# Pixie8888/R3DFSSeg

Hardware: AMD Instinct MI355X
Metric: episodes/sec S3DIS 2-way 5-shot 2048-pt (MPTI+attention, train step: forward+backward+grad all-reduce+Adam) (higher is better)
Workload: dtype f32 (index-free GEMMs -- self-attention, 1x1 convolutions, weight gradients, the EdgeConv backward's edge GEMMs -- as bf16x3 split products on the bf16 MFMA with fp32 accumulate; every index-deciding result: fp32)

## Files before the change

r3dfsseg_amd/csrc/head_graph.hip:

```cpp
#include "common.h"

#define HG_NC 4
typedef unsigned short hg_col_t;
#define HG_ROWS_PER_BLOCK_MIN 4
#define HG_MAX_PART 2048

struct HgEp {
  long nodes, nbr, y, z, g, lam, dn;
  long desc;
  long ws;
  long stats;
  long labels, logits, loss, pred;
};
#define HG_WS(p) p = (decltype(p))((const char*)(p) + (long)ep * st.ws * 4)
#define HG_AT(p, stride) p += (long)ep * (stride)

__global__ __launch_bounds__(256) void r3d_graph_bits_kernel(const int* __restrict__ nbr, int kp1, const int* __restrict__ n_dev,
                                                             int n_cap, int words, unsigned* __restrict__ outb, HgEp st) {
  __shared__ unsigned bm[4][1024];
  const int ep = blockIdx.y;
  nbr += (long)ep * st.nbr * kp1; HG_AT(n_dev, st.desc); HG_WS(outb);
  const int n = min(*n_dev, n_cap);
  const int w = threadIdx.x >> 6, lane = threadIdx.x & 63;
  const int i = blockIdx.x * 4 + w;
  unsigned* b = bm[w];
  for (int wd = lane; wd < words; wd += 64) b[wd] = 0u;
  __syncthreads();
  if (i < n) {
    const int k = kp1 - 1;
    for (int t = lane; t < k; t += 64) {
      const int j = nbr[(long)i * kp1 + 1 + t];
      if (j < 0 || j >= n || j == i) continue;
      atomicOr(&b[j >> 5], 1u << (j & 31));
    }
  }
  __syncthreads();
  if (i < n_cap)
    for (int wd = lane; wd < words; wd += 64) outb[(long)i * words + wd] = b[wd];
}

#define BT_ROWS 1024
#define BT_CW 8
__global__ __launch_bounds__(256) void r3d_graph_transpose_kernel(const unsigned* __restrict__ outb, int words, int n_cap,
                                                                  unsigned* __restrict__ inb ,
                                                                  HgEp st) {
  __shared__ unsigned tile[BT_CW * 32][BT_ROWS / 32 + 1];
  const int ep = blockIdx.z;
  HG_WS(outb); HG_WS(inb);
  const int c0w = blockIdx.x * BT_CW, r0 = blockIdx.y * BT_ROWS;
  const int w = threadIdx.x >> 6, lane = threadIdx.x & 63;
  for (int sb = w; sb < BT_ROWS / 64; sb += 4) {
    const int r = r0 + sb * 64 + lane;
    unsigned v[BT_CW];
#pragma unroll
    for (int cw = 0; cw < BT_CW; ++cw) v[cw] = (r < n_cap && c0w + cw < words) ? outb[(long)r * words + c0w + cw] : 0u;
#pragma unroll
    for (int cw = 0; cw < BT_CW; ++cw) {
#pragma unroll
      for (int b = 0; b < 32; ++b) {
        const unsigned long long m = __ballot((v[cw] >> b) & 1u);
        if (lane == b) {
          tile[cw * 32 + b][2 * sb] = (unsigned)m;
          tile[cw * 32 + b][2 * sb + 1] = (unsigned)(m >> 32);
        }
      }
    }
  }
  __syncthreads();
  for (int e = threadIdx.x; e < BT_CW * 32 * (BT_ROWS / 32); e += 256) {
    const int c = e >> 5, wd = e & 31;
    const int col = c0w * 32 + c, ow = r0 / 32 + wd;
    if (col < n_cap && ow < words) inb[(long)col * words + ow] = tile[c][wd];
  }
}

__global__ void r3d_graph_rowlen_kernel(unsigned* __restrict__ sym ,
                                        const unsigned* __restrict__ outb, int words,
                                        const int* __restrict__ n_dev, int n_cap, int* __restrict__ row_len, HgEp st) {
  const int ep = blockIdx.y;
  HG_WS(sym); HG_WS(outb); HG_AT(n_dev, st.desc); HG_WS(row_len);
  const int n = min(*n_dev, n_cap);
  const int row = blockIdx.x * (blockDim.x >> 6) + (threadIdx.x >> 6);
  const int lane = threadIdx.x & 63;
  if (row >= n_cap) return;
  int c = 0;
  if (row < n)
    for (int wd = lane; wd < words; wd += 64) {
      const unsigned v = sym[(long)row * words + wd] | outb[(long)row * words + wd];
      sym[(long)row * words + wd] = v;
      c += __popc(v);
    }
#pragma unroll
  for (int o = 32; o > 0; o >>= 1) c += __shfl_xor(c, o);
  if (lane == 0) row_len[row] = c;
}

__global__ __launch_bounds__(1024) void r3d_scan_kernel(const int* __restrict__ in, int n, int* __restrict__ out, HgEp st) {
  const int ep = blockIdx.x;
  HG_WS(in); HG_WS(out);
  __shared__ int wave_tot[16];
  __shared__ int carry_s;
  const int tid = threadIdx.x, lane = tid & 63, w = tid >> 6;
  if (tid == 0) carry_s = 0;
  __syncthreads();
  for (int t0 = 0; t0 < n; t0 += 1024) {
    const int i = t0 + tid;
    const int v = i < n ? in[i] : 0;
    int x = v;
#pragma unroll
    for (int o = 1; o < 64; o <<= 1) {
      const int y = __shfl_up(x, o);
      if (lane >= o) x += y;
    }
    if (lane == 63) wave_tot[w] = x;
    __syncthreads();
    int wbase = 0, tot = 0;
    for (int q = 0; q < 16; ++q) {
      const int tv = wave_tot[q];
      if (q < w) wbase += tv;
      tot += tv;
    }
    const int carry = carry_s;
    if (i < n) out[i] = carry + wbase + x - v;
    __syncthreads();
    if (tid == 0) carry_s = carry + tot;
    __syncthreads();
  }
  if (tid == 0) out[n] = carry_s;
}

__global__ __launch_bounds__(256) void r3d_graph_cols_kernel(const unsigned* __restrict__ sym, int words,
                                                             const int* __restrict__ n_dev, int n_cap,
                                                             const int* __restrict__ row_ptr, hg_col_t* __restrict__ col,
                                                             HgEp st) {
  const int ep = blockIdx.y;
  HG_WS(sym); HG_AT(n_dev, st.desc); HG_WS(row_ptr); HG_WS(col);
  const int n = min(*n_dev, n_cap);
  const int i = blockIdx.x * 4 + (threadIdx.x >> 6);
  const int lane = threadIdx.x & 63;
  if (i >= n) return;
  const int wpl = (words + 63) / 64;
  const int w0 = lane * wpl;
  int mycount = 0;
  for (int t = 0; t < wpl; ++t) {
    const int wd = w0 + t;
    if (wd < words) mycount += __popc(sym[(long)i * words + wd]);
  }
  int incl = mycount;
#pragma unroll
  for (int o = 1; o < 64; o <<= 1) {
    const int y = __shfl_up(incl, o);
    if (lane >= o) incl += y;
  }
  int wpos = row_ptr[i] + incl - mycount;
  for (int t = 0; t < wpl; ++t) {
    const int wd = w0 + t;
    if (wd >= words) break;
    unsigned bits = sym[(long)i * words + wd];
    while (bits) {
      const int b = __ffs((int)bits) - 1;
      bits &= bits - 1;
      col[wpos++] = (hg_col_t)(wd * 32 + b);
    }
  }
}

__global__ __launch_bounds__(256) void r3d_graph_weights_kernel(
    const float* __restrict__ nodes, long ldn, int D, const unsigned* __restrict__ outb, int words,
    const int* __restrict__ n_dev, int n_cap, const int* __restrict__ row_ptr, const hg_col_t* __restrict__ col,
    float sigma, float* __restrict__ val, float* __restrict__ dinv, float* __restrict__ wdir , HgEp st) {
  __shared__ __attribute__((aligned(16))) float xs[256];
  __shared__ float wsum[4];
  const int ep = blockIdx.y;
  nodes += (long)ep * st.nodes * ldn; HG_WS(outb); HG_AT(n_dev, st.desc); HG_WS(row_ptr); HG_WS(col); HG_WS(val); HG_WS(dinv);
  HG_WS(wdir);
  const int n = min(*n_dev, n_cap);
  const int w = threadIdx.x >> 6;
  const int i = blockIdx.x;
  const int lane = threadIdx.x & 63;
  if (i >= n) return;
  const float* xi = nodes + (long)i * ldn;
  xs[threadIdx.x] = (int)threadIdx.x < D ? xi[threadIdx.x] : 0.f;
  __syncthreads();
  const int beg = row_ptr[i], end = row_ptr[i + 1];
  const int D4 = D >> 2;
  const int part = lane & 7, slot = lane >> 3;
  float dsum = 0.f;
  for (int e0 = beg + 8 * w; e0 < end; e0 += 32) {
    const int e = e0 + slot;
    const bool ok = e < end;
    const int j = col[min(e, end - 1)];
    const float* xj = nodes + (long)j * ldn;
    float a = 0.f, b = 0.f;
    auto step = [&](const float4 y, int c4) {
      const float4 x = *reinterpret_cast<const float4*>(&xs[4 * c4]);
      float d1, d2;
      d1 = (x.x - y.x) + 1e-6f; d2 = (y.x - x.x) + 1e-6f; a = __builtin_fmaf(d1, d1, a); b = __builtin_fmaf(d2, d2, b);
      d1 = (x.y - y.y) + 1e-6f; d2 = (y.y - x.y) + 1e-6f; a = __builtin_fmaf(d1, d1, a); b = __builtin_fmaf(d2, d2, b);
      d1 = (x.z - y.z) + 1e-6f; d2 = (y.z - x.z) + 1e-6f; a = __builtin_fmaf(d1, d1, a); b = __builtin_fmaf(d2, d2, b);
      d1 = (x.w - y.w) + 1e-6f; d2 = (y.w - x.w) + 1e-6f; a = __builtin_fmaf(d1, d1, a); b = __builtin_fmaf(d2, d2, b);
    };
    int c4 = part;
    for (; c4 + 40 < D4; c4 += 48) {
      float4 y[6];
#pragma unroll
      for (int u = 0; u < 6; ++u) y[u] = *reinterpret_cast<const float4*>(xj + 4 * (c4 + 8 * u));
#pragma unroll
      for (int u = 0; u < 6; ++u) step(y[u], c4 + 8 * u);
    }
    for (; c4 < D4; c4 += 8) step(*reinterpret_cast<const float4*>(xj + 4 * c4), c4);
    if (part == 0) {
      for (int c = 4 * D4; c < D; ++c) {
        const float y = xj[c], x = xs[c];
        const float d1 = (x - y) + 1e-6f, d2 = (y - x) + 1e-6f;
        a = __builtin_fmaf(d1, d1, a);
        b = __builtin_fmaf(d2, d2, b);
      }
    }
    a = r3d_sum8_dpp(a);
    b = r3d_sum8_dpp(b);
    const bool out_ij = (outb[(long)i * words + (j >> 5)] >> (j & 31)) & 1u;
    const bool out_ji = (outb[(long)j * words + (i >> 5)] >> (i & 31)) & 1u;
    float wij = 0.f, wji = 0.f;
    if (out_ij) { const float d = sqrtf(a) / sigma; wij = expf(-0.5f * (d * d)); }
    if (out_ji) { const float d = sqrtf(b) / sigma; wji = expf(-0.5f * (d * d)); }
    const float wgt = wij + wji;
    if (ok && part == 0) {
      val[e] = wgt;
      *reinterpret_cast<float2*>(wdir + 2L * e) = make_float2(wij, wji);
      dsum += wgt;
    }
  }
  dsum = r3d_wave_sum(dsum);
  if (lane == 0) wsum[w] = dsum;
  __syncthreads();
  if (threadIdx.x == 0)
    dinv[i] = sqrtf(1.0f / ((((wsum[0] + wsum[1]) + wsum[2]) + wsum[3]) + 2.220446049250313e-16f));
}

__global__ void r3d_graph_normalize_kernel(const int* __restrict__ row_ptr, const hg_col_t* __restrict__ col,
                                           const float* __restrict__ dinv, const int* __restrict__ n_dev,
                                           int n_cap, float* __restrict__ val, HgEp st) {
  const int ep = blockIdx.y;
  HG_WS(row_ptr); HG_WS(col); HG_WS(dinv); HG_AT(n_dev, st.desc); HG_WS(val);
  const int n = min(*n_dev, n_cap);
  const int i = blockIdx.x * 4 + (threadIdx.x >> 6);
  const int lane = threadIdx.x & 63;
  if (i >= n) return;
  const float di = dinv[i];
  for (int e = row_ptr[i] + lane; e < row_ptr[i + 1]; e += 64) val[e] = (di * val[e]) * dinv[col[e]];
}

#define HG_MAX_ITER 1022
#define HG_M 64
#define HG_UROWS 256
#define HG_EBLOCKS 16
#define HG_PART (4 + 2 * HG_M * HG_NC)
static_assert(HG_M == 64 && HG_M * HG_NC == 256, "the CG kernels map (aggregate, column) onto 256 threads, aggregate = lane");
struct CgState {
  int done;
  int iters;
  unsigned ticket;
  unsigned ticket_k;
  float bb[HG_NC];
  float rz[HG_NC];
  float beta[HG_NC];
  float mu[HG_M * HG_NC];
  int fail;
  int pad_;
  unsigned long long pub[HG_M * HG_NC + HG_NC + 1];
};
#define CG_PUB_BETA (HG_M * HG_NC)
#define CG_PUB_CONV (HG_M * HG_NC + HG_NC)
#define CG_SPIN_LIMIT (1 << 18)
static_assert(offsetof(CgState, pub) % 8 == 0 && sizeof(CgState) % 4 == 0, "CgState: the published words are 8-byte words");

static __device__ __forceinline__ float4 f4_zero() { return make_float4(0.f, 0.f, 0.f, 0.f); }

static __device__ __forceinline__ float4 block_sum4(float4 v, float4* sm ) {
  const int lane = threadIdx.x & 63, w = threadIdx.x >> 6;
#pragma unroll
  for (int o = 32; o > 0; o >>= 1) {
    v.x += __shfl_xor(v.x, o); v.y += __shfl_xor(v.y, o);
    v.z += __shfl_xor(v.z, o); v.w += __shfl_xor(v.w, o);
  }
  __syncthreads();
  if (lane == 0) sm[w] = v;
  __syncthreads();
  const float4* sh = sm + (w & ~3);
  float4 r = sh[0];
  for (int q = 1; q < 4; ++q) { r.x += sh[q].x; r.y += sh[q].y; r.z += sh[q].z; r.w += sh[q].w; }
  return r;
}

static __device__ __forceinline__ float4 reduce_partials(const float4* part, int nblk, float4* sm) {
  float4 a = f4_zero();
  for (int q0 = threadIdx.x & 255; q0 < nblk; q0 += 8 * 256) {
    float4 p[8];
#pragma unroll
    for (int u = 0; u < 8; ++u) {
      const int q = q0 + 256 * u;
      const bool ok = q < nblk;
      p[u] = part[min(q, nblk - 1)];
      p[u].x = r3d_keep(p[u].x, ok); p[u].y = r3d_keep(p[u].y, ok); p[u].z = r3d_keep(p[u].z, ok); p[u].w = r3d_keep(p[u].w, ok);
    }
#pragma unroll
    for (int u = 0; u < 8; ++u) { a.x += p[u].x; a.y += p[u].y; a.z += p[u].z; a.w += p[u].w; }
  }
  return block_sum4(a, sm);
}

static __device__ __forceinline__ float f4_get(const float4& v, int c) { return c == 0 ? v.x : c == 1 ? v.y : c == 2 ? v.z : v.w; }

#define HG_SEED_PITCH 257
__global__ __launch_bounds__(256) void r3d_cg_aggregate_kernel(const float* __restrict__ nodes, long ldn, int D,
                                                               const int* __restrict__ n_dev, const int* __restrict__ n_proto_dev,
                                                               int n_cap, int rows_per_wave, int* __restrict__ agg, HgEp st) {
  extern __shared__ float smem[];
  {
    const int ep = blockIdx.y;
    nodes += (long)ep * st.nodes * ldn; HG_AT(n_dev, st.desc); HG_AT(n_proto_dev, st.desc); HG_WS(agg);
  }
  const int pitch = D | 1;
  float* seeds = smem;
  float* xrow = smem + HG_M * pitch + (threadIdx.x >> 6) * D;
  const int n = min(*n_dev, n_cap);
  const int n_proto = max(1, min(*n_proto_dev, n));
  const int lane = threadIdx.x & 63, w = threadIdx.x >> 6;
  {
    const int D4 = D >> 2;
    for (int s0 = 0; s0 < HG_M; s0 += 16) {
      const int sd = s0 + (threadIdx.x >> 4), l16 = threadIdx.x & 15;
      const int src = (int)(((long)sd * (n_proto - 1)) / (HG_M - 1));
      const float4* row = reinterpret_cast<const float4*>(nodes + (long)src * ldn);
      float4 v[4];
#pragma unroll
      for (int u = 0; u < 4; ++u) v[u] = row[min(l16 + 16 * u, D4 - 1)];
#pragma unroll
      for (int u = 0; u < 4; ++u) {
        const int c4 = l16 + 16 * u;
        if (c4 < D4) {
          float* dst = seeds + sd * pitch + 4 * c4;
          dst[0] = v[u].x; dst[1] = v[u].y; dst[2] = v[u].z; dst[3] = v[u].w;
        }
      }
    }
  }
  const int row0 = (blockIdx.x * 4 + w) * rows_per_wave;
  float xr[4][4];
#pragma unroll
  for (int k = 0; k < 4; ++k)
#pragma unroll
    for (int u = 0; u < 4; ++u)
      xr[k][u] = nodes[(long)min(row0 + min(k, rows_per_wave - 1), n - 1) * ldn + min(lane + 64 * u, D - 1)];
  __syncthreads();
  for (int k = 0; k < rows_per_wave; ++k) {
    const int i = row0 + k;
    if (i >= n) break;
#pragma unroll
    for (int u = 0; u < 4; ++u)
      if (lane + 64 * u < D) xrow[lane + 64 * u] = k == 0 ? xr[0][u] : k == 1 ? xr[1][u] : k == 2 ? xr[2][u] : xr[3][u];
    float d2 = 0.f;
    const float* sp = seeds + lane * pitch;
    for (int c0 = 0; c0 < D; c0 += 16) {
      float xs_[16], ss_[16];
#pragma unroll
      for (int c = 0; c < 16; ++c) { xs_[c] = xrow[min(c0 + c, D - 1)]; ss_[c] = sp[min(c0 + c, D - 1)]; }
#pragma unroll
      for (int c = 0; c < 16; ++c) {
        const float df = c0 + c < D ? xs_[c] - ss_[c] : 0.f;
        d2 = __builtin_fmaf(df, df, d2);
      }
    }
    unsigned long long key = ((unsigned long long)__float_as_uint(d2) << 32) | (unsigned)lane;
#pragma unroll
    for (int o = 32; o > 0; o >>= 1) {
      const unsigned long long other = __shfl_xor(key, o);
      key = other < key ? other : key;
    }
    if (lane == 0) agg[i] = (int)(key & 63u);
    __builtin_amdgcn_wave_barrier();
  }
}

__global__ __launch_bounds__(256) void r3d_cg_mw_kernel(const int* __restrict__ row_ptr, const hg_col_t* __restrict__ col,
                                                        const float* __restrict__ val, const float* __restrict__ dinv,
                                                        const int* __restrict__ agg, const int* __restrict__ n_dev, int n_cap,
                                                        float alpha_lp, int rows_per_wave, float* __restrict__ MW, HgEp st) {
  __shared__ float2 pairs[4][256];
  {
// ... 788 lines not shown
      const int i = row_of(trow);
      const float4 beta = beta_s;
      const float4 ri = rs[i], pi = p[i], qi = q[i];
      if (fused) r[i] = ri;
      const float u = 1.f / dinv[i];
      const float4 m = mu_s[agg[i]];
      const float4 pn = make_float4((ri.x + u * m.x) + beta.x * pi.x, (ri.y + u * m.y) + beta.y * pi.y,
                                    (ri.z + u * m.z) + beta.z * pi.z, (ri.w + u * m.w) + beta.w * pi.w);
      const float4 qn = make_float4((ri.x + tot.x) + beta.x * qi.x, (ri.y + tot.y) + beta.y * qi.y,
                                    (ri.z + tot.z) + beta.z * qi.z, (ri.w + tot.w) + beta.w * qi.w);
      p[i] = pn;
      q[i] = qn;
      acc_pq = make_float4(pn.x * qn.x, pn.y * qn.y, pn.z * qn.z, pn.w * qn.w);
    }
    pq_s[SL_WAVES * trow + w] = acc_pq;
    __syncthreads();
    if (tid < SL_PASS_ROWS / 4) {
      const float4 a = pq_s[4 * tid], b2 = pq_s[4 * tid + 1], c2 = pq_s[4 * tid + 2], d2 = pq_s[4 * tid + 3];
      const float4 t = make_float4(((a.x + b2.x) + c2.x) + d2.x, ((a.y + b2.y) + c2.y) + d2.y, ((a.z + b2.z) + c2.z) + d2.z,
                                   ((a.w + b2.w) + c2.w) + d2.w);
      const int gidx = (c0 + tid) * n_wg + bx;
      if (gidx < n_part) part_pq[gidx] = t;
    }
    __syncthreads();
  }
}

#ifdef CG_STAMPS
__device__ unsigned long long g_cg_dbg[32];
#define CSTAMP(i) do { if (it == 3 && threadIdx.x == 0 && blockIdx.x == 0) g_cg_dbg[i] = __builtin_amdgcn_s_memtime(); } while (0)
#define CSTAMP_LAST(i) do { if (it == 3 && threadIdx.x == 0) g_cg_dbg[16 + i] = __builtin_amdgcn_s_memtime(); } while (0)
extern "C" int r3d_cg_debug_read(unsigned long long* out32) {
  return hipMemcpyFromSymbol(out32, HIP_SYMBOL(g_cg_dbg), sizeof(g_cg_dbg)) == hipSuccess ? 0 : 1;
}
#else
#define CSTAMP(i)
#define CSTAMP_LAST(i)
#endif

__global__ __launch_bounds__(256) void r3d_cg_update_kernel(
    const int* __restrict__ n_dev, int n_cap, int it, int nblk_pq, const float* __restrict__ dinv, const int* __restrict__ agg,
    const float* __restrict__ MW, const float4* __restrict__ p, const float4* __restrict__ q, float4* __restrict__ x,
    float4* __restrict__ r, const float4* __restrict__ part_pq, float* __restrict__ part, const float* __restrict__ Einv,
    float tol2, CgState* __restrict__ cg, HgEp st, long x_stride) {
  __shared__ float4 sm[4];
  __shared__ float4 rs[HG_UROWS];
  __shared__ float us[HG_UROWS];
  __shared__ int ag[HG_UROWS];
  __shared__ float4 wpart[2 * 4 * HG_M];
  __shared__ double d_s[HG_M * HG_NC];
  __shared__ float t_s[HG_M * HG_NC];
  __shared__ float rr_s[HG_NC];
  __shared__ int last_s;
  {
    const int ep = blockIdx.y;
    HG_AT(n_dev, st.desc); HG_WS(dinv); HG_WS(agg); HG_WS(MW); HG_WS(p); HG_WS(q); HG_AT(x, x_stride); HG_WS(r); HG_WS(part_pq);
    HG_WS(part); HG_WS(Einv); HG_WS(cg);
  }
  if (cg->done | cg->fail) return;
  if (it < 0) it = cg->iters;
  const int row0 = blockIdx.x * HG_UROWS;
  const int i = row0 + threadIdx.x;
  const int ic = min(i, n_cap - 1);
  float m[64];
  CSTAMP(0);
  cg_load_mw_column(MW, row0, n_cap, m);
  const float4 pi = p[ic], qi = q[ic];
  float4 xi = x[ic], ri = r[ic];
  const float dv = dinv[ic];
  const int av = agg[ic];
  const float4 rz = *reinterpret_cast<const float4*>(cg->rz);
  const int n = min(*n_dev, n_cap);
  const float4 pq = reduce_partials(part_pq, nblk_pq, sm);
  CSTAMP(1);
  float4 al;
  al.x = pq.x > 0.f ? rz.x / pq.x : 0.f;
  al.y = pq.y > 0.f ? rz.y / pq.y : 0.f;
  al.z = pq.z > 0.f ? rz.z / pq.z : 0.f;
  al.w = pq.w > 0.f ? rz.w / pq.w : 0.f;
  float u = 0.f;
  int a = 0;
  if (i < n) {
    xi.x += al.x * pi.x; xi.y += al.y * pi.y; xi.z += al.z * pi.z; xi.w += al.w * pi.w;
    ri.x -= al.x * qi.x; ri.y -= al.y * qi.y; ri.z -= al.z * qi.z; ri.w -= al.w * qi.w;
    x[i] = xi; r[i] = ri;
    u = 1.f / dv;
    a = av;
  } else {
    ri = f4_zero();
  }
  rs[threadIdx.x] = ri; us[threadIdx.x] = u; ag[threadIdx.x] = a;
  __syncthreads();
  CSTAMP(2);
  cg_block_partials(rs, us, ag, row0, n, m, true, part + (long)blockIdx.x * HG_PART, sm, wpart);
  CSTAMP(3);
  const bool last = cg_delivered_last(cg, gridDim.x, &last_s);
  CSTAMP(4);
  if (last) {
    CSTAMP_LAST(0);
    cg_reduce_step<false>(part, gridDim.x, Einv, 1, it + 1, tol2, cg, d_s, t_s, rr_s);
    CSTAMP_LAST(1);
  }
}

__global__ __launch_bounds__(1024) void r3d_logits_ce_kernel(const float4* __restrict__ Z, const float4* __restrict__ Z2,
                                                             const int* __restrict__ desc_nproto, int n_q, int N, int n_classes,
                                                             const long long* __restrict__ labels,
                                                             float* __restrict__ logits ,
                                                             float* __restrict__ loss_out, int* __restrict__ pred_out, HgEp st) {
  __shared__ float red[16];
  {
    const int ep = blockIdx.x;
    HG_AT(Z, st.z); HG_AT(desc_nproto, st.desc); HG_AT(logits, st.logits);
    if (Z2) HG_AT(Z2, st.z);
    if (labels) HG_AT(labels, st.labels);
    if (loss_out) HG_AT(loss_out, st.loss);
    if (pred_out) HG_AT(pred_out, st.pred);
  }
  const int n_proto = *desc_nproto;
  float acc = 0.f;
  for (int e = threadIdx.x; e < n_q * N; e += blockDim.x) {
    const int qi = e / N, p = e - qi * N;
    const float4 z = Z[n_proto + e];
    const float4 z2 = Z2 ? Z2[n_proto + e] : f4_zero();
    const float zv[8] = {z.x, z.y, z.z, z.w, z2.x, z2.y, z2.z, z2.w};
    float mx = zv[0];
    int am = 0;
    for (int c = 1; c < n_classes; ++c) if (zv[c] > mx) { mx = zv[c]; am = c; }
    float se = 0.f;
    for (int c = 0; c < n_classes; ++c) {
      logits[((long)qi * n_classes + c) * N + p] = zv[c];
      se += expf(zv[c] - mx);
    }
    if (labels) {
      const int lab = (int)labels[e];
      acc += (mx + logf(se)) - zv[lab];
    }
    if (pred_out) pred_out[e] = am;
  }
  acc = r3d_wave_sum(acc);
  if ((threadIdx.x & 63) == 0) red[threadIdx.x >> 6] = acc;
  __syncthreads();
  if (threadIdx.x == 0) {
    float t = 0.f;
    for (int w = 0; w < (int)(blockDim.x >> 6); ++w) t += red[w];
    if (loss_out) *loss_out = t / (float)(n_q * N);
  }
}

struct LpWs {
  unsigned *outb, *sym;
  int *row_len, *row_ptr, *agg;
  hg_col_t* col;
  float *val, *dinv, *wdir, *MW, *Epart, *part;
  float* Einv;
  float4 *r, *p, *q, *part_pq;
  CgState* cg;
  long words, total;
};

static inline long hg_vblocks(int n_cap) { return r3d_cdiv(n_cap, HG_UROWS); }

static LpWs lp_carve(int32_t* ws, int n_cap, int kp1) {
  LpWs L;
  L.words = (n_cap + 31) / 32;
  const long nnz_cap = 2L * n_cap * (kp1 - 1);
  int32_t* wp = ws;
  auto align4 = [&]() { wp += (4 - ((wp - ws) & 3)) & 3; };
  L.outb = (unsigned*)wp; wp += n_cap * L.words;
  L.sym = (unsigned*)wp; wp += n_cap * L.words;
  L.row_len = wp; wp += n_cap + 8;
  L.row_ptr = wp; wp += n_cap + 8;
  L.col = (hg_col_t*)wp; wp += (nnz_cap + 1) / 2;
  L.val = (float*)wp; wp += nnz_cap;
  L.wdir = (float*)wp; wp += 2 * nnz_cap;
  L.dinv = (float*)wp; wp += n_cap;
  L.agg = wp; wp += n_cap;
  align4();
  L.MW = (float*)wp; wp += (long)n_cap * HG_M;
  L.Epart = (float*)wp; wp += (long)HG_EBLOCKS * HG_M * HG_M;
  align4();
  L.Einv = (float*)wp; wp += (long)HG_M * HG_M;
  L.part = (float*)wp; wp += hg_vblocks(n_cap) * HG_PART;
  align4();
  L.r = (float4*)wp; wp += 4L * n_cap;
  L.p = (float4*)wp; wp += 4L * n_cap;
  L.q = (float4*)wp; wp += 4L * n_cap;
  L.part_pq = (float4*)wp; wp += 4L * HG_MAX_PART;
  L.cg = (CgState*)wp; wp += (sizeof(CgState) + 3) / 4;
  L.total = (wp - ws) + 64;
  return L;
}

extern "C" long r3d_lp_ws_words(int n_cap, int kp1) { return lp_carve(nullptr, n_cap, kp1).total; }

extern "C" int r3d_lp_ws_offsets(int n_cap, int kp1, long* out6) {
  R3D_REQUIRE(out6 && n_cap > 0 && kp1 >= 2, "r3d_lp_ws_offsets: bad arguments");
  const LpWs L = lp_carve(nullptr, n_cap, kp1);
  const int32_t* base = nullptr;
  out6[0] = (const int32_t*)L.row_ptr - base; out6[1] = (const int32_t*)L.col - base; out6[2] = (const int32_t*)L.val - base;
  out6[3] = (const int32_t*)L.dinv - base; out6[4] = (const int32_t*)L.agg - base; out6[5] = (const int32_t*)L.cg - base;
  return R3D_OK;
}

__global__ void r3d_weights_compare_kernel(const int* __restrict__ row_ptr, const int* __restrict__ n_dev, int n_cap,
                                           const float* __restrict__ wdir, const float* __restrict__ wdir2, long scratch_stride,
                                           int* __restrict__ mismatch, HgEp st) {
  const int ep = blockIdx.y;
  HG_WS(row_ptr); HG_AT(n_dev, st.desc); HG_WS(wdir);
  wdir2 += (long)ep * scratch_stride;
  const int n = min(*n_dev, n_cap);
  const long nnz2 = 2L * row_ptr[n];
  int bad = 0;
  for (long e = (long)blockIdx.x * blockDim.x + threadIdx.x; e < nnz2; e += (long)gridDim.x * blockDim.x)
    bad += __float_as_uint(wdir[e]) != __float_as_uint(wdir2[e]) ? 1 : 0;
  bad = (int)r3d_wave_sum((float)bad);
  if ((threadIdx.x & 63) == 0 && bad) atomicAdd(mismatch, bad);
}
extern "C" long r3d_graph_weights_verify_words(int n_cap, int kp1) {
  const long nnz_cap = 2L * n_cap * (kp1 - 1);
  return 2 * nnz_cap + nnz_cap + n_cap + 64;
}
extern "C" int r3d_graph_weights_verify(int n_ep, const float* nodes, long ldn, int D, const int32_t* n_dev, long desc_stride,
                                        int n_cap, int kp1, float sigma, int32_t* ws, long ws_words, long ws_stride,
                                        float* scratch, int32_t* mismatch_out, void* stream) {
  R3D_REQUIRE(nodes && n_dev && ws && scratch && mismatch_out, "r3d_graph_weights_verify: null pointer");
  R3D_REQUIRE(n_cap > 0 && kp1 >= 2 && ws_words >= r3d_lp_ws_words(n_cap, kp1) && n_ep >= 1 &&
                  (n_ep == 1 || ((ws_stride & 3) == 0 && ws_stride >= ws_words)),
              "r3d_graph_weights_verify: bad arguments");
  hipStream_t st = (hipStream_t)stream;
  const LpWs L = lp_carve(ws, n_cap, kp1);
  const long nnz_cap = 2L * n_cap * (kp1 - 1), per = r3d_graph_weights_verify_words(n_cap, kp1);
  for (int e = 0; e < n_ep; ++e) {
    HgEp one{};
    float* base = scratch + (long)e * per;
    int32_t* wse = ws + (long)e * ws_stride;
    const LpWs Le = lp_carve(wse, n_cap, kp1);
    hipLaunchKernelGGL(r3d_graph_weights_kernel, dim3(n_cap, 1), dim3(256), 0, st, nodes + (long)e * n_cap * ldn, ldn, D, Le.outb,
                       (int)Le.words, n_dev + (long)e * desc_stride, n_cap, Le.row_ptr, Le.col, sigma, base + 2 * nnz_cap,
                       base + 3 * nnz_cap, base, one);
  }
  HgEp ep{};
  ep.desc = desc_stride; ep.ws = ws_stride;
  hipLaunchKernelGGL(r3d_weights_compare_kernel, dim3(256, n_ep), dim3(256), 0, st, L.row_ptr, n_dev, n_cap, L.wdir, scratch, per,
                     mismatch_out, ep);
  R3D_LAUNCH_CHECK("r3d_graph_weights_verify");
  return R3D_OK;
}

__global__ void r3d_cg_stats_kernel(const CgState* __restrict__ cg, int* __restrict__ stats_out, HgEp st) {
  const int ep = blockIdx.x;
  HG_WS(cg); HG_AT(stats_out, st.stats);
  if (threadIdx.x == 0) { stats_out[0] = cg->fail ? 0 : cg->done; stats_out[1] = cg->iters; }
}

static int lp_coarse_space(const LpWs& L, const float* nodes, long ldn, int D, const int32_t* n_dev, const int32_t* n_proto_dev,
                           int n_cap, float alpha, int n_ep, const HgEp& ep, hipStream_t st) {
  const int agg_rpw = 4;
  const size_t agg_lds = ((size_t)HG_M * (D | 1) + 4 * D) * sizeof(float);
  static bool lds_opt_in = false;
  if (!lds_opt_in) {
    hipFuncSetAttribute((const void*)r3d_cg_aggregate_kernel, hipFuncAttributeMaxDynamicSharedMemorySize, 96 * 1024);
    lds_opt_in = true;
  }
  hipLaunchKernelGGL(r3d_cg_aggregate_kernel, dim3(r3d_cdiv(n_cap, 4 * agg_rpw), n_ep), dim3(256), agg_lds, st, nodes, ldn, D,
                     n_dev, n_proto_dev, n_cap, agg_rpw, L.agg, ep);
  hipLaunchKernelGGL(r3d_cg_mw_kernel, dim3(r3d_cdiv(n_cap, 4), n_ep), dim3(256), 0, st, L.row_ptr, L.col, L.val, L.dinv, L.agg,
                     n_dev, n_cap, alpha, 1, L.MW, ep);
  hipLaunchKernelGGL(r3d_cg_epart_kernel, dim3(HG_EBLOCKS, n_ep), dim3(128), 0, st, L.MW, L.dinv, L.agg, n_dev, n_cap, L.Epart,
                     ep);
  hipLaunchKernelGGL(r3d_cg_einv_kernel, dim3(n_ep), dim3(1024), 0, st, L.Epart, L.Einv, ep);
  return R3D_OK;
}

static int g_cg_lds_min_blocks = 256;
extern "C" int r3d_debug_set_cg_spmv_lds_min_blocks(int min_blocks) {
  const int old = g_cg_lds_min_blocks;
  g_cg_lds_min_blocks = min_blocks;
  return old;
}

static int cg_lds_slots(size_t lds_r) {
  static size_t asked = 0;
  static int slots = 0;
  if (lds_r != asked || !slots) {
    int per_cu = 0, dev = 0, cus = 0;
    if (hipOccupancyMaxActiveBlocksPerMultiprocessor(&per_cu, r3d_cg_spmv_lds_kernel, 64 * SL_WAVES, lds_r) == hipSuccess &&
        per_cu > 0 && hipGetDevice(&dev) == hipSuccess &&
        hipDeviceGetAttribute(&cus, hipDeviceAttributeMultiprocessorCount, dev) == hipSuccess && cus > 0)
      slots = per_cu * cus;
    else {
      (void)hipGetLastError();
      slots = 256;
    }
    asked = lds_r;
  }
  return slots;
}

static int lp_solve(const LpWs& L, const float* RHS, long rhs_stride, const int32_t* n_dev, int n_cap, float alpha, int max_iter,
                    float tol, float* X, long x_stride, int32_t* stats_out, int n_ep, const HgEp& ep, hipStream_t st) {
  const int nblk_v = (int)hg_vblocks(n_cap);
  int rpb = HG_ROWS_PER_BLOCK_MIN;
  while (r3d_cdiv(n_cap, rpb) > HG_MAX_PART) rpb += 4;
  const int nblk_s = r3d_cdiv(n_cap, rpb);
  R3D_REQUIRE(nblk_s <= HG_MAX_PART, "r3d_label_propagate: n_cap too large");
  float4* x = (float4*)X;
  const float tol2 = tol * tol;
  r3d_fill_words_ep(&L.cg->ticket, 0u, (long)((sizeof(CgState) - offsetof(CgState, ticket)) / 4), n_ep, ep.ws, st);
  for (int mode = 0; mode < 2; ++mode)
    hipLaunchKernelGGL(r3d_cg_init_kernel, dim3(nblk_v, n_ep), dim3(256), 0, st, (const float4*)RHS, L.dinv, L.agg, L.MW, n_dev,
                       n_cap, mode, x, L.r, L.p, L.q, L.part, L.Einv, tol2, L.cg, ep, rhs_stride, x_stride);
  const size_t lds_r = (size_t)n_cap * sizeof(float4);
  const bool use_lds = lds_r <= SL_MAX_LDS && rpb == HG_ROWS_PER_BLOCK_MIN && (long)n_ep * r3d_cdiv(n_cap, SL_ROWS) >= g_cg_lds_min_blocks;
  if (use_lds) {
    static size_t attr = 0;
    if (lds_r > attr) {
      hipError_t e = hipFuncSetAttribute((const void*)r3d_cg_spmv_lds_kernel, hipFuncAttributeMaxDynamicSharedMemorySize, (int)lds_r);
      R3D_REQUIRE(e == hipSuccess, "r3d_label_propagate: cannot reserve %zu B of LDS: %s", lds_r, hipGetErrorString(e));
      attr = lds_r;
    }
  }
  const int nblk_l = use_lds ? std::max(1, std::min(r3d_cdiv(n_cap, SL_ROWS), cg_lds_slots(lds_r) / n_ep)) : 0;
  const int nblk_pq = nblk_s;
  for (int it = 0; it < max_iter; ++it) {
    if (use_lds) {
      hipLaunchKernelGGL(r3d_cg_spmv_lds_kernel, dim3(nblk_l, n_ep), dim3(64 * SL_WAVES), lds_r, st, L.row_ptr, L.col, L.val, L.dinv,
                         L.agg, L.MW, n_dev, n_cap, alpha, it, SL_ROWS, L.r, L.p, L.q, L.part_pq, L.cg, ep, x, L.part, L.Einv, tol2,
                         nblk_pq, nblk_v, x_stride);
      continue;
    }
    hipLaunchKernelGGL(r3d_cg_spmv_kernel, dim3(nblk_s, n_ep), dim3(256), 0, st, L.row_ptr, L.col, L.val, L.dinv, L.agg, L.MW,
                       n_dev, n_cap, alpha, it, rpb, L.r, L.p, L.q, L.part_pq, L.cg, ep);
    hipLaunchKernelGGL(r3d_cg_update_kernel, dim3(nblk_v, n_ep), dim3(256), 0, st, n_dev, n_cap, it, nblk_pq, L.dinv, L.agg, L.MW,
                       L.p, L.q, x, L.r, L.part_pq, L.part, L.Einv, tol2, L.cg, ep, x_stride);
  }
  if (use_lds)
    hipLaunchKernelGGL(r3d_cg_update_kernel, dim3(nblk_v, n_ep), dim3(256), 0, st, n_dev, n_cap, -1, nblk_pq, L.dinv, L.agg, L.MW,
                       L.p, L.q, x, L.r, L.part_pq, L.part, L.Einv, tol2, L.cg, ep, x_stride);
  if (stats_out) hipLaunchKernelGGL(r3d_cg_stats_kernel, dim3(n_ep), dim3(64), 0, st, L.cg, stats_out, ep);
  return R3D_OK;
}

static int label_propagate_impl(int n_ep, const HgEp& ep, const float* nodes, long ldn, int D, const int32_t* nbr, int kp1,
                                const float* Y, const int32_t* n_dev, const int32_t* n_proto_dev, int n_cap, float sigma,
                                float alpha, int max_iter, float tol, float* Z, int32_t* ws, long ws_words, int32_t* stats_out,
                                void* stream) {
  R3D_REQUIRE(nodes && nbr && Y && n_dev && n_proto_dev && Z && ws, "r3d_label_propagate: null pointer");
  R3D_REQUIRE(n_cap > 0 && kp1 >= 2 && ws_words >= r3d_lp_ws_words(n_cap, kp1),
              "r3d_label_propagate: workspace of %ld words, r3d_lp_ws_words(%d, %d) = %ld needed", ws_words, n_cap, kp1,
              n_cap > 0 && kp1 >= 2 ? r3d_lp_ws_words(n_cap, kp1) : -1L);
  R3D_REQUIRE((ldn & 3) == 0 && ((uintptr_t)nodes & 15) == 0,
              "r3d_label_propagate: node rows are read as float4: ldn must be a multiple of 4 and nodes 16-byte aligned");
  R3D_REQUIRE(n_cap > 0 && n_cap <= 32768 && D > 0 && D <= 256 && (D & 3) == 0 && kp1 >= 2,
              "r3d_label_propagate: unsupported n_cap=%d D=%d kp1=%d", n_cap, D, kp1);
  R3D_REQUIRE(max_iter > 0 && max_iter <= HG_MAX_ITER && sigma > 0.f, "r3d_label_propagate: bad solver parameters");
  R3D_REQUIRE(((uintptr_t)ws & 15) == 0 && ((uintptr_t)Y & 15) == 0 && ((uintptr_t)Z & 15) == 0,
              "r3d_label_propagate: ws, Y and Z must be 16-byte aligned");
  R3D_REQUIRE(n_ep >= 1 && n_ep <= 4096 && (n_ep == 1 || ((ep.ws & 3) == 0 && ep.ws >= ws_words)),
              "r3d_label_propagate: %d systems need a scratch stride that is a multiple of 4 words and >= the scratch size", n_ep);
  hipStream_t st = (hipStream_t)stream;
  const LpWs L = lp_carve(ws, n_cap, kp1);
  const long words = L.words;
  hipLaunchKernelGGL(r3d_graph_bits_kernel, dim3(r3d_cdiv(n_cap, 4), n_ep), dim3(256), 0, st, nbr, kp1, n_dev, n_cap,
                     (int)words, L.outb, ep);
  hipLaunchKernelGGL(r3d_graph_transpose_kernel, dim3(r3d_cdiv(words, BT_CW), r3d_cdiv(n_cap, BT_ROWS), n_ep), dim3(256), 0, st,
                     L.outb, (int)words, n_cap, L.sym, ep);
  hipLaunchKernelGGL(r3d_graph_rowlen_kernel, dim3(r3d_cdiv(n_cap, 4), n_ep), dim3(256), 0, st, L.sym, L.outb, (int)words,
                     n_dev, n_cap, L.row_len, ep);
  hipLaunchKernelGGL(r3d_scan_kernel, dim3(n_ep), dim3(1024), 0, st, L.row_len, n_cap, L.row_ptr, ep);
  hipLaunchKernelGGL(r3d_graph_cols_kernel, dim3(r3d_cdiv(n_cap, 4), n_ep), dim3(256), 0, st, L.sym, (int)words, n_dev,
                     n_cap, L.row_ptr, L.col, ep);
  hipLaunchKernelGGL(r3d_graph_weights_kernel, dim3(n_cap, n_ep), dim3(256), 0, st, nodes, ldn, D, L.outb,
                     (int)words, n_dev, n_cap, L.row_ptr, L.col, sigma, L.val, L.dinv, L.wdir, ep);
  hipLaunchKernelGGL(r3d_graph_normalize_kernel, dim3(r3d_cdiv(n_cap, 4), n_ep), dim3(256), 0, st, L.row_ptr, L.col, L.dinv,
                     n_dev, n_cap, L.val, ep);
  int rc = lp_coarse_space(L, nodes, ldn, D, n_dev, n_proto_dev, n_cap, alpha, n_ep, ep, st);
  if (rc) return rc;
  rc = lp_solve(L, Y, ep.y, n_dev, n_cap, alpha, max_iter, tol, Z, ep.z, stats_out, n_ep, ep, st);
  if (rc) return rc;
  R3D_LAUNCH_CHECK("r3d_label_propagate");
  return R3D_OK;
}

extern "C" int r3d_label_propagate(const float* nodes, long ldn, int D, const int32_t* nbr, int kp1,
                                   const float* Y, const int32_t* n_dev, const int32_t* n_proto_dev, int n_cap, float sigma,
                                   float alpha, int max_iter, float tol, float* Z, int32_t* ws, long ws_words,
                                   int32_t* stats_out, void* stream) {
  const HgEp one{};
  return label_propagate_impl(1, one, nodes, ldn, D, nbr, kp1, Y, n_dev, n_proto_dev, n_cap, sigma, alpha, max_iter, tol, Z, ws,
                              ws_words, stats_out, stream);
}

extern "C" int r3d_label_propagate_solve_batched(int n_ep, const float* Y, const int32_t* n_dev, long desc_stride, int n_cap,
                                                 int kp1, float alpha, int max_iter, float tol, float* Z, int32_t* ws,
                                                 long ws_words, long ws_stride, int32_t* stats_out, long stats_stride,
                                                 void* stream) {
  R3D_REQUIRE(Y && n_dev && Z && ws, "r3d_label_propagate_solve: null pointer");
  R3D_REQUIRE(n_cap > 0 && kp1 >= 2 && ws_words >= r3d_lp_ws_words(n_cap, kp1), "r3d_label_propagate_solve: workspace too short");
  R3D_REQUIRE(max_iter > 0 && max_iter <= HG_MAX_ITER, "r3d_label_propagate_solve: bad solver parameters");
  R3D_REQUIRE(((uintptr_t)ws & 15) == 0 && ((uintptr_t)Y & 15) == 0 && ((uintptr_t)Z & 15) == 0,
              "r3d_label_propagate_solve: ws, Y and Z must be 16-byte aligned");
  R3D_REQUIRE(n_ep >= 1 && n_ep <= 4096 && (n_ep == 1 || ((ws_stride & 3) == 0 && ws_stride >= ws_words)),
              "r3d_label_propagate_solve: bad scratch stride");
  HgEp ep{};
  ep.nodes = ep.nbr = ep.y = ep.z = n_cap;
  ep.desc = desc_stride; ep.ws = ws_stride; ep.stats = stats_stride;
  const LpWs L = lp_carve(ws, n_cap, kp1);
  const int rc = lp_solve(L, Y, ep.y, n_dev, n_cap, alpha, max_iter, tol, Z, ep.z, stats_out, n_ep, ep, (hipStream_t)stream);
  if (rc) return rc;
  R3D_LAUNCH_CHECK("r3d_label_propagate_solve");
  return R3D_OK;
}

extern "C" int r3d_label_propagate_batched(int n_ep, const float* nodes, long ldn, int D, const int32_t* nbr, int kp1,
                                           const float* Y, const int32_t* n_dev, const int32_t* n_proto_dev, long desc_stride,
                                           int n_cap, float sigma, float alpha, int max_iter, float tol, float* Z, int32_t* ws,
                                           long ws_words, long ws_stride, int32_t* stats_out, long stats_stride, void* stream) {
  HgEp ep{};
  ep.nodes = ep.nbr = ep.y = ep.z = n_cap;
  ep.desc = desc_stride; ep.ws = ws_stride; ep.stats = stats_stride;
  return label_propagate_impl(n_ep, ep, nodes, ldn, D, nbr, kp1, Y, n_dev, n_proto_dev, n_cap, sigma, alpha, max_iter, tol, Z, ws,
                              ws_words, stats_out, stream);
}

static __device__ __forceinline__ float dot4(float4 a, float4 b) { return a.x * b.x + a.y * b.y + a.z * b.z + a.w * b.w; }

__global__ __launch_bounds__(256) void r3d_lp_bwd_dd_kernel(const int* __restrict__ row_ptr, const hg_col_t* __restrict__ col,
                                                            const float* __restrict__ val, const float* __restrict__ dinv,
                                                            const int* __restrict__ n_dev, int n_cap, float alpha,
                                                            const float4* __restrict__ lam, const float4* __restrict__ Z,
                                                            float* __restrict__ dD, HgEp st) {
  const int ep = blockIdx.y;
  HG_WS(row_ptr); HG_WS(col); HG_WS(val); HG_WS(dinv); HG_AT(n_dev, st.desc); HG_AT(lam, st.lam); HG_AT(Z, st.z); HG_WS(dD);
  const int n = min(*n_dev, n_cap);
  const int i = blockIdx.x * 4 + (threadIdx.x >> 6);
  const int lane = threadIdx.x & 63;
  if (i >= n) return;
  const float4 li = lam[i], zi = Z[i];
  const float di = dinv[i];
  float g = 0.f;
  for (int e = row_ptr[i] + lane; e < row_ptr[i + 1]; e += 64) {
    const int j = col[e];
    const float ds = alpha * (dot4(li, Z[j]) + dot4(lam[j], zi));
    g += ds * (val[e] / di);
  }
  g = r3d_wave_sum(g);
  if (lane == 0) dD[i] = -0.5f * di * di * di * g;
}

__global__ __launch_bounds__(256) void r3d_lp_bwd_dx_kernel(
    const float* __restrict__ nodes, long ldn, int D, const float* __restrict__ wdir,
    const int* __restrict__ row_ptr, const hg_col_t* __restrict__ col, const float* __restrict__ dinv,
    const int* __restrict__ n_dev, int n_cap, float sigma, float alpha, const float4* __restrict__ lam,
    const float4* __restrict__ Z, const float* __restrict__ dD, float* __restrict__ dnodes, long ldd, HgEp st) {
  {
    const int ep = blockIdx.y;
    nodes += (long)ep * st.nodes * ldn; HG_WS(wdir); HG_WS(row_ptr); HG_WS(col); HG_WS(dinv); HG_AT(n_dev, st.desc);
    HG_AT(lam, st.lam); HG_AT(Z, st.z); HG_WS(dD); dnodes += (long)ep * st.dn * ldd;
  }
  __shared__ float acc_s[4][256];
  __shared__ float uv_s[4][2];
  const int n = min(*n_dev, n_cap);
  const int w = threadIdx.x >> 6;
  const int i = blockIdx.x;
  const int lane = threadIdx.x & 63;
  if (i >= n) return;
  const float* xi = nodes + (long)i * ldn;
  const float4 li = lam[i], zi = Z[i];
  const float di = dinv[i], ddi = dD[i];
  const int beg = row_ptr[i], end = row_ptr[i + 1];
  const float inv_s2 = 1.f / (sigma * sigma);
  const int c0 = min(lane, D - 1), c1 = min(lane + 64, D - 1), c2 = min(lane + 128, D - 1), c3 = min(lane + 192, D - 1);
  float U = 0.f, V = 0.f;
  float a0 = 0.f, a1 = 0.f, a2 = 0.f, a3 = 0.f;
  for (int e0 = beg + 64 * w; e0 < end; e0 += 256) {
    const int e = e0 + lane;
    const bool ok = e < end;
    const int ec = min(e, end - 1);
    const int j = col[ec];
    const float2 wd = *reinterpret_cast<const float2*>(wdir + 2L * ec);
    const float dj = dinv[j];
    const float T = alpha * (dot4(li, Z[j]) + dot4(lam[j], zi)) * di * dj + ddi + dD[j];
    const float cij = ok ? -T * wd.x * inv_s2 : 0.f;
    const float cji = ok ? -T * wd.y * inv_s2 : 0.f;
    const float u = cij + cji;
    U += u;
    V += cij - cji;
    const int cnt = min(64, end - e0);
    int t = 0;
    for (; t + 8 <= cnt; t += 8) {
      float x0[8], x1[8], x2[8], x3[8], ut[8];
#pragma unroll
      for (int q = 0; q < 8; ++q) {
        ut[q] = r3d_readlane_f(u, t + q);
        const float* xr = nodes + (long)__builtin_amdgcn_readlane(j, t + q) * ldn;
        x0[q] = xr[c0]; x1[q] = xr[c1]; x2[q] = xr[c2];
        x3[q] = D > 192 ? xr[c3] : 0.f;
      }
#pragma unroll
      for (int q = 0; q < 8; ++q) {
        a0 = __builtin_fmaf(ut[q], x0[q], a0); a1 = __builtin_fmaf(ut[q], x1[q], a1);
        a2 = __builtin_fmaf(ut[q], x2[q], a2); a3 = __builtin_fmaf(ut[q], x3[q], a3);
      }
    }
    for (; t < cnt; ++t) {
      const float ut = r3d_readlane_f(u, t);
      const float* xr = nodes + (long)__builtin_amdgcn_readlane(j, t) * ldn;
      a0 = __builtin_fmaf(ut, xr[c0], a0); a1 = __builtin_fmaf(ut, xr[c1], a1);
      a2 = __builtin_fmaf(ut, xr[c2], a2); a3 = __builtin_fmaf(ut, D > 192 ? xr[c3] : 0.f, a3);
    }
  }
  U = r3d_wave_sum(U);
  V = r3d_wave_sum(V);
  acc_s[w][lane] = a0; acc_s[w][64 + lane] = a1; acc_s[w][128 + lane] = a2; acc_s[w][192 + lane] = a3;
  if (lane == 0) { uv_s[w][0] = U; uv_s[w][1] = V; }
  __syncthreads();
  const int c = threadIdx.x;
  if (c < D) {
    const float At = ((acc_s[0][c] + acc_s[1][c]) + acc_s[2][c]) + acc_s[3][c];
    const float Ut = ((uv_s[0][0] + uv_s[1][0]) + uv_s[2][0]) + uv_s[3][0];
    const float Vt = ((uv_s[0][1] + uv_s[1][1]) + uv_s[2][1]) + uv_s[3][1];
    dnodes[(long)i * ldd + c] = xi[c] * Ut - At + 1e-6f * Vt;
  }
}

__global__ void r3d_ce_grad_kernel(const float4* __restrict__ Z, const int* __restrict__ n_proto_dev, int n_cap, int n_qpts,
// ... 126 lines not shown
```

Before: 404.0.

## Compute symmetric graph edge weights once per pair and mirror them

The rowlen kernel now also stores a per-word prefix rank of the symmetric adjacency bits. A new pairs kernel uses that rank to find, for each edge i-j with j<i, the mirror edge slot in row j, computes the feature distance once and writes both directed weight pairs. A separate rowsum kernel then builds edge values and degree inverses. This roughly halves the distance computations in graph construction, at the cost of an extra rank array, an extra launch, and scattered writes to the mirror slots.

```diff
diff --git a/r3dfsseg_amd/csrc/head_graph.hip b/r3dfsseg_amd/csrc/head_graph.hip
--- a/r3dfsseg_amd/csrc/head_graph.hip
+++ b/r3dfsseg_amd/csrc/head_graph.hip
@@ -76,22 +76,29 @@
 
 __global__ void r3d_graph_rowlen_kernel(unsigned* __restrict__ sym ,
                                         const unsigned* __restrict__ outb, int words,
-                                        const int* __restrict__ n_dev, int n_cap, int* __restrict__ row_len, HgEp st) {
+                                        const int* __restrict__ n_dev, int n_cap, int* __restrict__ row_len,
+                                        hg_col_t* __restrict__ rank ,
+                                        HgEp st) {
   const int ep = blockIdx.y;
-  HG_WS(sym); HG_WS(outb); HG_AT(n_dev, st.desc); HG_WS(row_len);
+  HG_WS(sym); HG_WS(outb); HG_AT(n_dev, st.desc); HG_WS(row_len); HG_WS(rank);
   const int n = min(*n_dev, n_cap);
   const int row = blockIdx.x * (blockDim.x >> 6) + (threadIdx.x >> 6);
   const int lane = threadIdx.x & 63;
   if (row >= n_cap) return;
   int c = 0;
   if (row < n)
-    for (int wd = lane; wd < words; wd += 64) {
-      const unsigned v = sym[(long)row * words + wd] | outb[(long)row * words + wd];
-      sym[(long)row * words + wd] = v;
-      c += __popc(v);
-    }
-#pragma unroll
-  for (int o = 32; o > 0; o >>= 1) c += __shfl_xor(c, o);
+    for (int w0 = 0; w0 < words; w0 += 64) {
+      const int wd = w0 + lane;
+      unsigned v = 0u;
+      if (wd < words) {
+        v = sym[(long)row * words + wd] | outb[(long)row * words + wd];
+        sym[(long)row * words + wd] = v;
+      }
+      const int pc = __popc(v);
+      const int incl = r3d_wave_incl_scan(pc);
+      if (wd < words) rank[(long)row * words + wd] = (hg_col_t)(c + incl - pc);
+      c += __shfl(incl, 63);
+    }
   if (lane == 0) row_len[row] = c;
 }
 
@@ -165,6 +172,44 @@
   }
 }
 
+
+static __device__ __forceinline__ void hg_pair_dist2(const float* xs, const float* __restrict__ xj, int D, int part, float& a,
+                                                     float& b) {
+  const int D4 = D >> 2;
+  a = 0.f; b = 0.f;
+  auto step = [&](const float4 y, int c4) {
+    const float4 x = *reinterpret_cast<const float4*>(&xs[4 * c4]);
+    float d1, d2;
+    d1 = (x.x - y.x) + 1e-6f; d2 = (y.x - x.x) + 1e-6f; a = __builtin_fmaf(d1, d1, a); b = __builtin_fmaf(d2, d2, b);
+    d1 = (x.y - y.y) + 1e-6f; d2 = (y.y - x.y) + 1e-6f; a = __builtin_fmaf(d1, d1, a); b = __builtin_fmaf(d2, d2, b);
+    d1 = (x.z - y.z) + 1e-6f; d2 = (y.z - x.z) + 1e-6f; a = __builtin_fmaf(d1, d1, a); b = __builtin_fmaf(d2, d2, b);
+    d1 = (x.w - y.w) + 1e-6f; d2 = (y.w - x.w) + 1e-6f; a = __builtin_fmaf(d1, d1, a); b = __builtin_fmaf(d2, d2, b);
+  };
+  int c4 = part;
+  for (; c4 + 40 < D4; c4 += 48) {
+    float4 y[6];
+#pragma unroll
+    for (int u = 0; u < 6; ++u) y[u] = *reinterpret_cast<const float4*>(xj + 4 * (c4 + 8 * u));
+#pragma unroll
+    for (int u = 0; u < 6; ++u) step(y[u], c4 + 8 * u);
+  }
+  for (; c4 < D4; c4 += 8) step(*reinterpret_cast<const float4*>(xj + 4 * c4), c4);
+  if (part == 0) {
+    for (int c = 4 * D4; c < D; ++c) {
+      const float y = xj[c], x = xs[c];
+      const float d1 = (x - y) + 1e-6f, d2 = (y - x) + 1e-6f;
+      a = __builtin_fmaf(d1, d1, a);
+      b = __builtin_fmaf(d2, d2, b);
+    }
+  }
+  a = r3d_sum8_dpp(a);
+  b = r3d_sum8_dpp(b);
+}
+static __device__ __forceinline__ float hg_gauss(float dist2, float sigma) {
+  const float d = sqrtf(dist2) / sigma;
+  return expf(-0.5f * (d * d));
+}
+
 __global__ __launch_bounds__(256) void r3d_graph_weights_kernel(
     const float* __restrict__ nodes, long ldn, int D, const unsigned* __restrict__ outb, int words,
     const int* __restrict__ n_dev, int n_cap, const int* __restrict__ row_ptr, const hg_col_t* __restrict__ col,
@@ -183,47 +228,17 @@
   xs[threadIdx.x] = (int)threadIdx.x < D ? xi[threadIdx.x] : 0.f;
   __syncthreads();
   const int beg = row_ptr[i], end = row_ptr[i + 1];
-  const int D4 = D >> 2;
   const int part = lane & 7, slot = lane >> 3;
   float dsum = 0.f;
   for (int e0 = beg + 8 * w; e0 < end; e0 += 32) {
     const int e = e0 + slot;
     const bool ok = e < end;
     const int j = col[min(e, end - 1)];
-    const float* xj = nodes + (long)j * ldn;
-    float a = 0.f, b = 0.f;
-    auto step = [&](const float4 y, int c4) {
-      const float4 x = *reinterpret_cast<const float4*>(&xs[4 * c4]);
-      float d1, d2;
-      d1 = (x.x - y.x) + 1e-6f; d2 = (y.x - x.x) + 1e-6f; a = __builtin_fmaf(d1, d1, a); b = __builtin_fmaf(d2, d2, b);
-      d1 = (x.y - y.y) + 1e-6f; d2 = (y.y - x.y) + 1e-6f; a = __builtin_fmaf(d1, d1, a); b = __builtin_fmaf(d2, d2, b);
-      d1 = (x.z - y.z) + 1e-6f; d2 = (y.z - x.z) + 1e-6f; a = __builtin_fmaf(d1, d1, a); b = __builtin_fmaf(d2, d2, b);
-      d1 = (x.w - y.w) + 1e-6f; d2 = (y.w - x.w) + 1e-6f; a = __builtin_fmaf(d1, d1, a); b = __builtin_fmaf(d2, d2, b);
-    };
-    int c4 = part;
-    for (; c4 + 40 < D4; c4 += 48) {
-      float4 y[6];
-#pragma unroll
-      for (int u = 0; u < 6; ++u) y[u] = *reinterpret_cast<const float4*>(xj + 4 * (c4 + 8 * u));
-#pragma unroll
-      for (int u = 0; u < 6; ++u) step(y[u], c4 + 8 * u);
-    }
-    for (; c4 < D4; c4 += 8) step(*reinterpret_cast<const float4*>(xj + 4 * c4), c4);
-    if (part == 0) {
-      for (int c = 4 * D4; c < D; ++c) {
-        const float y = xj[c], x = xs[c];
-        const float d1 = (x - y) + 1e-6f, d2 = (y - x) + 1e-6f;
-        a = __builtin_fmaf(d1, d1, a);
-        b = __builtin_fmaf(d2, d2, b);
-      }
-    }
-    a = r3d_sum8_dpp(a);
-    b = r3d_sum8_dpp(b);
+    float a, b;
+    hg_pair_dist2(xs, nodes + (long)j * ldn, D, part, a, b);
     const bool out_ij = (outb[(long)i * words + (j >> 5)] >> (j & 31)) & 1u;
     const bool out_ji = (outb[(long)j * words + (i >> 5)] >> (i & 31)) & 1u;
-    float wij = 0.f, wji = 0.f;
-    if (out_ij) { const float d = sqrtf(a) / sigma; wij = expf(-0.5f * (d * d)); }
-    if (out_ji) { const float d = sqrtf(b) / sigma; wji = expf(-0.5f * (d * d)); }
+    const float wij = out_ij ? hg_gauss(a, sigma) : 0.f, wji = out_ji ? hg_gauss(b, sigma) : 0.f;
     const float wgt = wij + wji;
     if (ok && part == 0) {
       val[e] = wgt;
@@ -236,6 +251,72 @@
   __syncthreads();
   if (threadIdx.x == 0)
     dinv[i] = sqrtf(1.0f / ((((wsum[0] + wsum[1]) + wsum[2]) + wsum[3]) + 2.220446049250313e-16f));
+}
+
+__global__ __launch_bounds__(256) __attribute__((amdgpu_waves_per_eu(7, 8))) void r3d_graph_pairs_kernel(
+    const float* __restrict__ nodes, long ldn, int D, const unsigned* __restrict__ outb, const unsigned* __restrict__ sym,
+    const hg_col_t* __restrict__ rank, int words, const int* __restrict__ n_dev, int n_cap, const int* __restrict__ row_ptr,
+    const hg_col_t* __restrict__ col, float sigma, int nnz_cap, float* __restrict__ wdir , HgEp st) {
+  __shared__ __attribute__((aligned(16))) float xs[256];
+  const int ep = blockIdx.y;
+  nodes += (long)ep * st.nodes * ldn; HG_WS(outb); HG_WS(sym); HG_WS(rank); HG_AT(n_dev, st.desc); HG_WS(row_ptr); HG_WS(col);
+  HG_WS(wdir);
+  const int n = min(*n_dev, n_cap);
+  const int w = threadIdx.x >> 6;
+  const int i = blockIdx.x;
+  const int lane = threadIdx.x & 63;
+  if (i >= n) return;
+  const int iw = i >> 5;
+  const unsigned below = (1u << (i & 31)) - 1u;
+  const int own = rank[(long)i * words + iw] + __popc(sym[(long)i * words + iw] & below);
+  if (own == 0) return;
+  const float* xi = nodes + (long)i * ldn;
+  xs[threadIdx.x] = (int)threadIdx.x < D ? xi[threadIdx.x] : 0.f;
+  __syncthreads();
+  const int beg = row_ptr[i], lim = beg + own;
+  const int part = lane & 7, slot = lane >> 3;
+  for (int e0 = beg + 8 * w; e0 < lim; e0 += 32) {
+    const int e = e0 + slot;
+    const bool ok = e < lim;
+    const int j = col[min(e, lim - 1)];
+    const long jw = (long)j * words + iw;
+    const unsigned o_i = outb[(long)i * words + (j >> 5)], o_j = outb[jw], s_j = sym[jw];
+    const int e2 = row_ptr[j] + rank[jw] + __popc(s_j & below);
+    float a, b;
+    hg_pair_dist2(xs, nodes + (long)j * ldn, D, part, a, b);
+    const bool out_ij = (o_i >> (j & 31)) & 1u;
+    const bool out_ji = (o_j >> (i & 31)) & 1u;
+    const float wij = out_ij ? hg_gauss(a, sigma) : 0.f, wji = out_ji ? hg_gauss(b, sigma) : 0.f;
+    if (ok && part == 0 && e2 < nnz_cap) {
+      *reinterpret_cast<float2*>(wdir + 2L * e) = make_float2(wij, wji);
+      *reinterpret_cast<float2*>(wdir + 2L * e2) = make_float2(wji, wij);
+    }
+  }
+}
+
+__global__ __launch_bounds__(256) void r3d_graph_rowsum_kernel(const int* __restrict__ row_ptr, const float* __restrict__ wdir,
+                                                               const int* __restrict__ n_dev, int n_cap, float* __restrict__ val,
+                                                               float* __restrict__ dinv, HgEp st) {
+  const int ep = blockIdx.y;
+  HG_WS(row_ptr); HG_WS(wdir); HG_WS(val); HG_AT(n_dev, st.desc); HG_WS(dinv);
+  const int n = min(*n_dev, n_cap);
+  const int i = blockIdx.x * 4 + (threadIdx.x >> 6);
+  const int lane = threadIdx.x & 63;
+  if (i >= n) return;
+  const int beg = row_ptr[i], end = row_ptr[i + 1];
+  float s = 0.f;
+  if (lane < 32)
+    for (int e = beg + lane; e < end; e += 32) {
+      const float2 wd = *reinterpret_cast<const float2*>(wdir + 2L * e);
+      const float wgt = wd.x + wd.y;
+      val[e] = wgt;
+      s += wgt;
+    }
+  s += __shfl_xor(s, 4);
+  s += __shfl_xor(s, 2);
+  s += __shfl_xor(s, 1);
+  const float w0 = __shfl(s, 0), w1 = __shfl(s, 8), w2 = __shfl(s, 16), w3 = __shfl(s, 24);
+  if (lane == 0) dinv[i] = sqrtf(1.0f / ((((w0 + w1) + w2) + w3) + 2.220446049250313e-16f));
 }
 
 __global__ void r3d_graph_normalize_kernel(const int* __restrict__ row_ptr, const hg_col_t* __restrict__ col,
@@ -1330,6 +1411,7 @@
   unsigned *outb, *sym;
   int *row_len, *row_ptr, *agg;
   hg_col_t* col;
+  hg_col_t* rank;
   float *val, *dinv, *wdir, *MW, *Epart, *part;
   float* Einv;
   float4 *r, *p, *q, *part_pq;
@@ -1366,6 +1448,8 @@
   L.q = (float4*)wp; wp += 4L * n_cap;
   L.part_pq = (float4*)wp; wp += 4L * HG_MAX_PART;
   L.cg = (CgState*)wp; wp += (sizeof(CgState) + 3) / 4;
+  align4();
+  L.rank = (hg_col_t*)wp; wp += ((long)n_cap * L.words + 1) / 2;
   L.total = (wp - ws) + 64;
   return L;
 }
@@ -1545,12 +1629,14 @@
   hipLaunchKernelGGL(r3d_graph_transpose_kernel, dim3(r3d_cdiv(words, BT_CW), r3d_cdiv(n_cap, BT_ROWS), n_ep), dim3(256), 0, st,
                      L.outb, (int)words, n_cap, L.sym, ep);
   hipLaunchKernelGGL(r3d_graph_rowlen_kernel, dim3(r3d_cdiv(n_cap, 4), n_ep), dim3(256), 0, st, L.sym, L.outb, (int)words,
-                     n_dev, n_cap, L.row_len, ep);
+                     n_dev, n_cap, L.row_len, L.rank, ep);
   hipLaunchKernelGGL(r3d_scan_kernel, dim3(n_ep), dim3(1024), 0, st, L.row_len, n_cap, L.row_ptr, ep);
   hipLaunchKernelGGL(r3d_graph_cols_kernel, dim3(r3d_cdiv(n_cap, 4), n_ep), dim3(256), 0, st, L.sym, (int)words, n_dev,
                      n_cap, L.row_ptr, L.col, ep);
-  hipLaunchKernelGGL(r3d_graph_weights_kernel, dim3(n_cap, n_ep), dim3(256), 0, st, nodes, ldn, D, L.outb,
-                     (int)words, n_dev, n_cap, L.row_ptr, L.col, sigma, L.val, L.dinv, L.wdir, ep);
+  hipLaunchKernelGGL(r3d_graph_pairs_kernel, dim3(n_cap, n_ep), dim3(256), 0, st, nodes, ldn, D, L.outb, L.sym, L.rank,
+                     (int)words, n_dev, n_cap, L.row_ptr, L.col, sigma, (int)(2L * n_cap * (kp1 - 1)), L.wdir, ep);
+  hipLaunchKernelGGL(r3d_graph_rowsum_kernel, dim3(r3d_cdiv(n_cap, 4), n_ep), dim3(256), 0, st, L.row_ptr, L.wdir, n_dev, n_cap,
+                     L.val, L.dinv, ep);
   hipLaunchKernelGGL(r3d_graph_normalize_kernel, dim3(r3d_cdiv(n_cap, 4), n_ep), dim3(256), 0, st, L.row_ptr, L.col, L.dinv,
                      n_dev, n_cap, L.val, ep);
   int rc = lp_coarse_space(L, nodes, ldn, D, n_dev, n_proto_dev, n_cap, alpha, n_ep, ep, st);
```

Result: no change. 407.3, median of 4 (+0.8%).
